# pwrliang/grpc-rdma

Measured on NVIDIA H100. Metric: streaming_payload_GBps_256conns_4MiB, higher is better.
Workload: dtype u8

## Files before the change

grpc-rdma_b200/csrc/b200_block.cuh:

```cuda
#pragma once
#include <cuda_runtime.h>
#include <stdint.h>

#include "b200_dev.cuh"
#include "b200_warp.cuh"

#ifndef VL
#define VL(x) (*(volatile decltype(x)*)&(x))
#endif

#ifndef B200_RECV_PROXY_FENCE
#define B200_RECV_PROXY_FENCE 1
#endif

namespace b200 {


__device__ __forceinline__ uint32_t smem_u32(const void* p) { return (uint32_t)__cvta_generic_to_shared(p); }
__device__ __forceinline__ void mbar_init(uint64_t* bar, uint32_t count) {
  asm volatile("mbarrier.init.shared::cta.b64 [%0], %1;" ::"r"(smem_u32(bar)), "r"(count) : "memory");
}
__device__ __forceinline__ void mbar_expect_tx(uint64_t* bar, uint32_t bytes) {
  asm volatile("mbarrier.arrive.expect_tx.shared::cta.b64 _, [%0], %1;" ::"r"(smem_u32(bar)), "r"(bytes) : "memory");
}
// ... 1 lines not shown
  uint32_t ok;
  asm volatile(
      "{\n\t.reg .pred p;\n\t"
      "mbarrier.try_wait.parity.shared::cta.b64 p, [%1], %2;\n\t"
      "selp.u32 %0, 1, 0, p;\n\t}"
      : "=r"(ok)
      : "r"(smem_u32(bar)), "r"(parity)
      : "memory");
  return ok != 0;
}
__device__ __forceinline__ void bulk_g2s(void* sdst, const void* gsrc, uint32_t bytes, uint64_t* bar) {
  asm volatile("cp.async.bulk.shared::cluster.global.mbarrier::complete_tx::bytes [%0], [%1], %2, [%3];" ::"r"(
                   smem_u32(sdst)),
               "l"(gsrc), "r"(bytes), "r"(smem_u32(bar))
               : "memory");
}
__device__ __forceinline__ void fence_proxy_async_global() { asm volatile("fence.proxy.async.global;" ::: "memory"); }
__device__ __forceinline__ void bulk_s2g(void* gdst, const void* ssrc, uint32_t bytes) {
  asm volatile("cp.async.bulk.global.shared::cta.bulk_group [%0], [%1], %2;" ::"l"(gdst), "r"(smem_u32(ssrc)),
               "r"(bytes)
               : "memory");
}
__device__ __forceinline__ void bulk_commit() { asm volatile("cp.async.bulk.commit_group;" ::: "memory"); }

template <int K>
__device__ __forceinline__ void realign_vectors(uint4* sv, uint32_t nvec, uint32_t r, uint32_t lane) {
  for (uint32_t j = 0; j < nvec; j += 32) {
    const uint32_t i = j + lane;
    uint4 o = make_uint4(0, 0, 0, 0);
    if (i < nvec) {
      const uint4 A = sv[i], B = sv[i + 1];
      uint32_t x0, x1, x2, x3, x4;
      if (K == 0) { x0 = A.x; x1 = A.y; x2 = A.z; x3 = A.w; x4 = B.x; }
      else if (K == 1) { x0 = A.y; x1 = A.z; x2 = A.w; x3 = B.x; x4 = B.y; }
      else if (K == 2) { x0 = A.z; x1 = A.w; x2 = B.x; x3 = B.y; x4 = B.z; }
      else { x0 = A.w; x1 = B.x; x2 = B.y; x3 = B.z; x4 = B.w; }
      o.x = __funnelshift_r(x0, x1, r);
      o.y = __funnelshift_r(x1, x2, r);
      o.z = __funnelshift_r(x2, x3, r);
      o.w = __funnelshift_r(x3, x4, r);
    }
    __syncwarp();
    if (i < nvec) sv[i] = o;
  }
}

__device__ __forceinline__ void smem_to_global(uint8_t* dst, uint8_t* sbase, uint32_t soff, uint32_t n,
                                               uint32_t lane) {
  if (n == 0) return;
  uint32_t head = (16 - (uint32_t)(reinterpret_cast<uintptr_t>(dst) & 15)) & 15;
  if (head > n) head = n;
  const uint32_t nvec = (n - head) >> 4;
  const uint32_t tail = n - head - (nvec << 4);
  if (lane < head) dst[lane] = sbase[soff + lane];
  if (lane < tail) dst[head + (nvec << 4) + lane] = sbase[soff + head + (nvec << 4) + lane];
  if (nvec == 0) return;
  const uint32_t vs = soff + head, m = vs & 15;
  uint4* sv = reinterpret_cast<uint4*>(sbase + (vs - m));
  if (m != 0) {
    __syncwarp();
    const uint32_t r = (m & 3) * 8;
    switch (m >> 2) {
      case 0: realign_vectors<0>(sv, nvec, r, lane); break;
      case 1: realign_vectors<1>(sv, nvec, r, lane); break;
      case 2: realign_vectors<2>(sv, nvec, r, lane); break;
      default: realign_vectors<3>(sv, nvec, r, lane); break;
    }
    asm volatile("fence.proxy.async.shared::cta;" ::: "memory");
    __syncwarp();
  }
  if (lane == 0) bulk_s2g(dst + head, sv, nvec << 4);
}

constexpr uint32_t kZeroBytes = 1024;
__device__ __forceinline__ void coop_zero(uint8_t* p, uint64_t n, const uint8_t* zero, uint32_t lane) {
  if (n == 0) return;
  uint64_t head = (16 - (reinterpret_cast<uintptr_t>(p) & 15)) & 15;
  if (head > n) head = n;
  if (lane < head) p[lane] = 0;
  p += head;
  n -= head;
  const uint64_t body = n & ~15ull;
  if (lane < n - body) p[body + lane] = 0;
  if (lane == 0)
    for (uint64_t o = 0; o < body; o += kZeroBytes)
      bulk_s2g(p + o, zero, body - o < kZeroBytes ? (uint32_t)(body - o) : kZeroBytes);
}


#ifndef B200_MOVERS
#define B200_MOVERS 8
#endif
#ifndef B200_DEPTH
#define B200_DEPTH 3
// ... 110 lines not shown
      bulk_commit();
      *(volatile uint32_t*)&w->ready = 0;
    }
    head++;
  }
  if (lane == 0) {
    asm volatile("cp.async.bulk.wait_group 0;" ::: "memory");
    fence_proxy_async_global();
  }
  __syncwarp();
}


constexpr uint32_t kTiny = 32;
constexpr uint32_t kFootCap = 1024;
__device__ __forceinline__ void foot_put(uint32_t* foot8, bool stamped, uint32_t i, uint64_t off, uint64_t p) {
  if (stamped) reinterpret_cast<uint64_t*>(foot8)[i] = (off >> 3) | p << 32;
  else foot8[i] = (uint32_t)(off >> 3);
}

struct SendPlanState {
  uint64_t rt, cap, staging, total_left, written_total, ncalls, cur, bidx, last_rh;
  uint64_t tx;
  uint32_t partial, max_sge, coalesce, stamped;
};

struct SendCallScratch {
  const uint8_t* src[kMaxSgeLimit];
  uint64_t len[kMaxSgeLimit];
  uint64_t off[kMaxSgeLimit];
  uint32_t first_item[kMaxSgeLimit + 1];
};

template <bool kStamped>
__device__ __noinline__ void send_produce_segment(const SendOpDev& op, const PairDev* P, uint8_t* ring,
                                                  SendPlanState& S, SendCallScratch& CS, WorkItem* q, PipeCtl* ctl,
                                                  uint32_t* foot8, uint32_t* nfoot_out, uint32_t lane) {
  const uint64_t cap = S.cap, mask = cap - 1;
  uint32_t base_item = 0, nfoot = 0;
  bool op_done = false;
  constexpr bool stamped = kStamped;
  const uint32_t fcap = stamped ? kFootCap / 2 : kFootCap;
  while (nfoot + kMaxSgeLimit <= fcap) {
    const uint64_t rt = S.rt, tx0 = S.tx;
    const uint64_t rh = ld_volatile_u64(&P->credit_head);
    if (rh != S.last_rh) {
      if (P->wire != 0) __threadfence_system();
      else __threadfence();
      S.last_rh = rh;
    }
    const uint64_t cur = S.cur, bidx = S.bidx;
    const uint64_t idx = cur + lane;
    const bool valid = lane < S.max_sge && idx < op.nreal;
    const uint8_t* ptr = nullptr;
    uint64_t len = 0;
    if (valid) {
      SliceDev sl = op.slices[idx];
      const uint64_t skip = lane == 0 ? bidx : 0;
      ptr = sl.ptr + skip;
      len = sl.len - skip;
    }
    const uint64_t e = valid ? encoded_size(len) : 0;
// ... 12 lines not shown
    const int nfull = first_bad < 0 ? 32 : first_bad;
    uint64_t p = 0;
    if ((int)lane < nfull) p = len;
    else if ((int)lane == nfull && valid && len != 0) p = room;
    const unsigned fmask = __ballot_sync(0xffffffffu, p != 0);
    const uint32_t nframes = __popc(fmask);
    uint64_t wsum = p, esum = p ? encoded_size(p) : 0;
    const bool tiny = p != 0 && p <= kTiny;
    const uint32_t items = (p && !tiny) ? (uint32_t)((p + kChunk - 1) / kChunk) : 0;
    uint32_t items_incl = items;
    for (int o = 1; o < 32; o <<= 1) {
      uint32_t t = __shfl_up_sync(0xffffffffu, items_incl, o);
      if (lane >= (uint32_t)o) items_incl += t;
    }
    for (int o = 16; o > 0; o >>= 1) {
      wsum += __shfl_xor_sync(0xffffffffu, wsum, o);
      esum += __shfl_xor_sync(0xffffffffu, esum, o);
    }
    const uint32_t nitems = __shfl_sync(0xffffffffu, items_incl, 31);
    const uint64_t cut_p = __shfl_sync(0xffffffffu, p, nfull < 32 ? nfull : 0);
    const uint64_t foff = (rt + a) & mask;
    const uint64_t hdr = frame_header(p, stamped ? stamp_of(tx0 + lane) : 0);
    CS.first_item[lane] = items_incl - items;
    if (p) {
      CS.src[lane] = ptr;
      CS.len[lane] = p;
      CS.off[lane] = foff;
      foot_put(foot8, stamped, nfoot + lane, (foff + 8 + round_up8(p)) & mask, p);
    }
    if (tiny) {
      uint64_t w[kTiny / 8];
#pragma unroll
      for (int k = 0; k < (int)(kTiny / 8); k++) w[k] = 0;
#pragma unroll
      for (int i = 0; i < (int)kTiny; i++)
        if ((uint64_t)i < p) w[i >> 3] |= (uint64_t)__ldg(ptr + i) << (8 * (i & 7));
      *reinterpret_cast<uint64_t*>(ring + foff) = hdr;
#pragma unroll
      for (int k = 0; k < (int)(kTiny / 8); k++)
        if ((uint64_t)(8 * k) < p) *reinterpret_cast<uint64_t*>(ring + ((foff + 8 + 8 * k) & mask)) = w[k];
    }
    if (lane == 0) {
      CS.first_item[32] = nitems;
      S.rt = (rt + esum) & mask;
      S.tx = tx0 + nframes;
      S.partial = wsum < S.total_left;
      S.total_left -= wsum;
      S.written_total += wsum;
      if (wsum) S.ncalls++;
      uint64_t nb = 0;
      if (nfull < 32 && nframes > (uint32_t)nfull) nb = (nfull == 0 ? bidx : 0) + cut_p;
      else if (nfull == 0) nb = bidx;
      S.cur = cur + nfull;
      S.bidx = nb;
    }
    __syncwarp();
    nfoot += nframes;
    const unsigned big = __ballot_sync(0xffffffffu, items > 8);
    if (!big && nitems <= kQI) {
      const uint32_t first = items_incl - items;
      for (uint32_t t = 0; t < items; t++) {
        const uint64_t c0 = (uint64_t)t * kChunk;
        uint64_t n = p - c0;
        if (n > kChunk) n = kChunk;
        publish_item(q, base_item + first + t, reinterpret_cast<uint64_t>(ptr + c0), (foff + 8 + c0) & mask,
                     c0 == 0 ? hdr : 0, (uint32_t)n);
      }
    } else
    for (uint32_t it = lane; it < nitems; it += 32) {
      uint32_t f = 0;
      while (f + 1 < nframes && CS.first_item[f + 1] <= it) f++;
      const uint64_t c0 = (uint64_t)(it - CS.first_item[f]) * kChunk;
      const uint64_t flen = CS.len[f];
      uint64_t n = flen - c0;
      if (n > kChunk) n = kChunk;
      publish_item(q, base_item + it, reinterpret_cast<uint64_t>(CS.src[f] + c0), (CS.off[f] + 8 + c0) & mask,
                   c0 == 0 ? frame_header(flen, stamped ? stamp_of(tx0 + f) : 0) : 0, (uint32_t)n);
    }
    __syncwarp();
    base_item += nitems;
    const bool last = (wsum == 0) || !(op.flags & kFlagUntilBlocked) || S.total_left == 0;
    if (last) {
      op_done = true;
      break;
    }
  }
  if (lane == 0) {
    *nfoot_out = nfoot;
    ctl->total_items = base_item;
    ctl->op_done = op_done ? 1u : 0u;
    __threadfence_block();
    *(volatile uint32_t*)&ctl->seg_done = 1;
  }
  __syncwarp();
}

template <bool kStamped>
__device__ __noinline__ void send_produce_coalesced(const SendOpDev& op, const PairDev* P, uint8_t* ring,
                                                    SendPlanState& S, SendCallScratch& CS, WorkItem* q, PipeCtl* ctl,
                                                    uint32_t* foot8, uint32_t* nfoot_out, uint32_t lane) {
  const uint64_t cap = S.cap, mask = cap - 1;
  uint32_t base_item = 0, nfoot = 0;
  bool op_done = false;
  constexpr bool stamped = kStamped;
  const uint32_t fcap = stamped ? kFootCap / 2 : kFootCap;
  while (nfoot < fcap) {
    const uint64_t rt = S.rt;
    const uint64_t rh = ld_volatile_u64(&P->credit_head);
    if (rh != S.last_rh) {
      if (P->wire != 0) __threadfence_system();
      else __threadfence();
      S.last_rh = rh;
    }
    const uint64_t cur = S.cur, bidx = S.bidx;
    const uint64_t wend = op.nreal < cur + kCoalesceSlices ? op.nreal : cur + kCoalesceSlices;
    const uint64_t ws = calc_writable(S.staging), wf = calc_writable(free_size(cap, rh, rt));
    const uint64_t pmax = ws < wf ? ws : wf;
    uint64_t p = 0;
    for (uint64_t g = cur; g < wend && p < pmax; g += 32) {
      const uint64_t idx = g + lane;
      uint64_t len = idx < wend ? op.slices[idx].len - (idx == cur ? bidx : 0) : 0;
      for (int o = 16; o > 0; o >>= 1) len += __shfl_xor_sync(0xffffffffu, len, o);
      p += len;
    }
    if (p > pmax) p = pmax;
// ... 20 lines not shown
      passed += __popc(__ballot_sync(0xffffffffu, valid && a < p && e <= p));
      const unsigned cm = __ballot_sync(0xffffffffu, valid && a < p && e > p);
      if (cm) {
        nb = __shfl_sync(0xffffffffu, skip + (p - a), __ffs(cm) - 1);
        cut = true;
      }
      const bool tiny = n != 0 && n <= kTiny;
      const uint32_t items = (n && !tiny) ? (uint32_t)((n + kChunk - 1) / kChunk) : 0;
      uint32_t items_incl = items;
      for (int o = 1; o < 32; o <<= 1) {
        const uint32_t t = __shfl_up_sync(0xffffffffu, items_incl, o);
        if (lane >= (uint32_t)o) items_incl += t;
      }
      const uint32_t nitems = __shfl_sync(0xffffffffu, items_incl, 31);
      const uint64_t foff = (rt + 8 + a) & mask;
      if (tiny) {
#pragma unroll 1
        for (uint32_t i = 0; i < (uint32_t)n; i++) ring[(foff + i) & mask] = __ldg(ptr + i);
      }
      CS.first_item[lane] = items_incl - items;
      CS.src[lane] = ptr;
      CS.len[lane] = n;
      CS.off[lane] = foff;
      __syncwarp();
      for (uint32_t it = lane; it < nitems; it += 32) {
        uint32_t f = 0;
        while (f + 1 < 32 && CS.first_item[f + 1] <= it) f++;
        const uint64_t c0 = (uint64_t)(it - CS.first_item[f]) * kChunk;
        uint64_t m = CS.len[f] - c0;
        if (m > kChunk) m = kChunk;
        publish_item(q, base_item + it, reinterpret_cast<uint64_t>(CS.src[f] + c0), (CS.off[f] + c0) & mask, 0,
                     (uint32_t)m);
      }
      __syncwarp();
      base_item += nitems;
      pre = __shfl_sync(0xffffffffu, e, 31);
    }
    if (lane == 0) {
      if (p) {
        *reinterpret_cast<uint64_t*>(ring + rt) = frame_header(p, stamped ? stamp_of(S.tx) : 0);
        foot_put(foot8, stamped, nfoot, (rt + 8 + round_up8(p)) & mask, p);
        S.tx++;
        S.rt = (rt + encoded_size(p)) & mask;
        S.ncalls++;
        S.cur = cur + passed;
        S.bidx = cut ? nb : 0;
      }
      S.partial = p < S.total_left;
      S.total_left -= p;
      S.written_total += p;
    }
    __syncwarp();
    if (p) nfoot++;
    if (p == 0 || !(op.flags & kFlagUntilBlocked) || S.total_left == 0) {
      op_done = true;
      break;
    }
  }
  if (lane == 0) {
    *nfoot_out = nfoot;
    ctl->total_items = base_item;
    ctl->op_done = op_done ? 1u : 0u;
    __threadfence_block();
    *(volatile uint32_t*)&ctl->seg_done = 1;
  }
  __syncwarp();
}

struct SendMove {
  uint8_t* ring;
  uint64_t cap, mask;
  __device__ __forceinline__ void issue(uint64_t a, uint32_t n, uint8_t* stage, uint64_t* bar) const {
    const uint32_t pre = (uint32_t)(a & 15);
    const uint32_t len = (pre + n + 15u) & ~15u;
    mbar_expect_tx(bar, len);
    bulk_g2s(stage, reinterpret_cast<const void*>(a - pre), len, bar);
  }
  __device__ __forceinline__ void process(uint64_t a, uint64_t b, uint64_t c, uint32_t n, uint8_t* stage,
                                          uint32_t lane) const {
    const uint32_t pre = (uint32_t)(a & 15);
    if (c != 0 && lane == 0) *reinterpret_cast<uint64_t*>(ring + ((b + cap - 8) & mask)) = c;
    uint64_t seg1 = cap - b;
    if (seg1 > n) seg1 = n;
    smem_to_global(ring + b, stage, pre, (uint32_t)seg1, lane);
    if (n > seg1) smem_to_global(ring, stage, pre + (uint32_t)seg1, n - (uint32_t)seg1, lane);
  }
};

__device__ __forceinline__ void send_body(PairDev* __restrict__ pairs, const SendOpDev& op, OpResult* result,
                                          PipeSmem& pipe, uint8_t* stage_mem, uint32_t& phase_bits) {
  WorkItem* q = pipe.q;
  PipeCtl& ctl = pipe.ctl;
  uint64_t* bars = pipe.bars;
  __shared__ SendPlanState PS;
  __shared__ SendCallScratch CS;
  __shared__ uint64_t foot_mem[kFootCap / 2];
  uint32_t* foot8 = reinterpret_cast<uint32_t*>(foot_mem);
  __shared__ uint32_t s_nfoot;
  __shared__ unsigned long long s_tx0;
  __shared__ unsigned long long s_total;
  __shared__ uint32_t s_status;
  PairDev* P = &pairs[op.slot];
  const uint32_t tid = threadIdx.x, lane = tid & 31, warp = tid >> 5;

  if (tid < kQI) q[tid].ready = 0;
  if (tid == 0) {
    s_total = 0;
    s_status = *(volatile uint32_t*)&P->status;
    PS.rt = *(volatile uint64_t*)&P->remote_tail;
    PS.cap = *(volatile uint64_t*)&P->cap;
    PS.staging = PS.cap / 2;
    const uint32_t sge = *(volatile uint32_t*)&P->max_sge;
    PS.max_sge = sge & ~kSgeModeBits;
    PS.coalesce = (sge & kSgeCoalesce) != 0;
    PS.stamped = (sge & kSgeStamped) != 0;
    PS.tx = PS.stamped ? VL(pair_seq(pairs, op.slot)->tx) : 0;
    PS.cur = 0;
    PS.bidx = op.byte_idx;
    PS.written_total = 0;
    PS.ncalls = 0;
    PS.partial = *(volatile uint32_t*)&P->partial_write;
    PS.last_rh = ~0ull;
  }
  __syncthreads();
  {
    unsigned long long part = 0;
    for (uint64_t i = tid; i < op.nslices; i += kThreads) part += op.slices[i].len;
    for (int o = 16; o > 0; o >>= 1) part += __shfl_down_sync(0xffffffffu, part, o);
    if (lane == 0 && part) atomicAdd(&s_total, part);
  }
  __syncthreads();
  if (s_status != kStConnected) {
    if (tid == 0) {
      result->bytes = 0;
      result->calls = 0;
    }
    return;
  }
  if (tid == 0) PS.total_left = s_total - op.byte_idx;
  const uint64_t cap = VL(P->cap), mask = cap - 1;
  uint8_t* ring = VL(P->peer_ring);
  const bool sys_scope = VL(P->wire) != 0;

  while (true) {
    if (tid == 0) {
      ctl.next = 0;
      ctl.total_items = 0;
      ctl.seg_done = 0;
      ctl.op_done = 0;
      s_nfoot = 0;
      s_tx0 = PS.tx;
    }
    __syncthreads();
    if (warp == 0) {
      if (PS.stamped) {
        if (PS.coalesce) send_produce_coalesced<true>(op, P, ring, PS, CS, q, &ctl, foot8, &s_nfoot, lane);
        else send_produce_segment<true>(op, P, ring, PS, CS, q, &ctl, foot8, &s_nfoot, lane);
      } else {
        if (PS.coalesce) send_produce_coalesced<false>(op, P, ring, PS, CS, q, &ctl, foot8, &s_nfoot, lane);
        else send_produce_segment<false>(op, P, ring, PS, CS, q, &ctl, foot8, &s_nfoot, lane);
      }
    } else {
      const SendMove mv{ring, cap, mask};
      mover_run(mv, q, &ctl, stage_mem + (warp - 1) * (kDepth * kStageBytes), &bars[(warp - 1) * kDepth], phase_bits, lane);
    }
    if (sys_scope) __threadfence_system();
    else __threadfence();
    __syncthreads();
    const uint32_t nfoot = s_nfoot;
    if (PS.stamped) {
      for (uint32_t i = tid; i < nfoot; i += kThreads) {
        const uint64_t v = foot_mem[i];
        const uint64_t hdr = frame_header(v >> 32, stamp_of(s_tx0 + i));
        *reinterpret_cast<uint64_t*>(ring + ((v & 0xffffffffu) << 3)) = ~hdr;
      }
    } else {
      for (uint32_t i = tid; i < nfoot; i += kThreads)
        *reinterpret_cast<uint64_t*>(ring + ((uint64_t)foot8[i] << 3)) = kFooter;
    }
    const bool done = ctl.op_done != 0;
    __syncthreads();
    if (done) break;
  }
  if (tid == 0) {
    P->remote_tail = PS.rt;
    P->partial_write = PS.partial;
    if (PS.stamped) pair_seq(pairs, op.slot)->tx = PS.tx;
// ... 410 lines not shown
```

grpc-rdma_b200/csrc/b200_dev.cuh:

```cuda
#pragma once
#include <stdint.h>

#if defined(__CUDACC__)
#define B200_HD __host__ __device__ __forceinline__
#else
#define B200_HD inline
#endif

namespace b200 {

constexpr uint64_t kAlign = 8;
constexpr uint64_t kReserved = 24;
constexpr uint64_t kFooter = ~0ull;
constexpr int kMaxSgeLimit = 32;
constexpr uint32_t kCoalesceSlices = 1024;
constexpr uint32_t kSgeCoalesce = 0x80000000u;
constexpr uint32_t kSgeStamped = 0x40000000u;
constexpr uint32_t kSgeModeBits = kSgeCoalesce | kSgeStamped;
constexpr uint64_t kStampMod = (1ull << 24) - 1;
constexpr uint64_t kLenMask = (1ull << 40) - 1;
constexpr uint64_t kStampedMaxCap = 256ull << 20;
constexpr int kMaxPairs = 8192;

B200_HD uint64_t round_up8(uint64_t v) { return (v + 7) & ~7ull; }
B200_HD uint64_t round_down8(uint64_t v) { return v & ~7ull; }
B200_HD uint64_t encoded_size(uint64_t payload) { return 16 + round_up8(payload); }
B200_HD uint64_t calc_writable(uint64_t space) { return space > kReserved ? round_down8(space - kReserved) : 0; }
B200_HD uint64_t free_size(uint64_t cap, uint64_t head, uint64_t tail) {
  return cap - ((tail + cap - head) & (cap - 1));
}
B200_HD uint64_t writable_size(uint64_t cap, uint64_t head, uint64_t tail) {
  uint64_t f = free_size(cap, head, tail);
  return f > kReserved ? f - kReserved : 0;
}

B200_HD uint32_t stamp_of(uint64_t s) { return 1u + (uint32_t)(s % kStampMod); }
B200_HD uint64_t frame_header(uint64_t p, uint32_t st) { return p | (uint64_t)st << 40; }
B200_HD uint64_t frame_footer(uint64_t hdr, uint32_t st) { return st ? ~hdr : kFooter; }
B200_HD uint64_t frame_present(uint64_t hdr, uint64_t cap, uint32_t st) {
  const uint64_t p = st ? hdr & kLenMask : hdr;
  if (st && (uint32_t)(hdr >> 40) != st) return 0;
  return p != 0 && p <= cap - kReserved ? p : 0;
}
B200_HD uint64_t frame_complete(uint64_t hdr, uint64_t foot, uint64_t cap, uint32_t st) {
  const uint64_t p = frame_present(hdr, cap, st);
// ... 140 lines not shown
  uint16_t events;
};
struct SvcPollState {
  uint32_t hi_slot;
  uint32_t stop;
  uint32_t ready_next;
  uint32_t scans;
};
struct SvcParams {
  PairDev* pairs;
  PairSvc* psvc;
  SvcCmd* cmds;
  SvcDone* done;
  BigBox* boxes;
  EagerRec* erec;
  uint8_t* eslots;
  SvcPollState* ps;
  uint32_t* last_ev;
  ReadyEntry* ready;
  uint32_t* host_scans;
  int nowners, nbig;
};

void launch_send(PairDev* pairs, const SendOpDev* ops, OpResult* results, int nops, void* stream);
void launch_recv(PairDev* pairs, const RecvOpDev* ops, OpResult* results, int nops, void* stream);
void launch_poll_scan(PairDev* pairs, const int32_t* slots, uint32_t* events, uint32_t* ready_count,
                      int32_t* ready_slots, int n, void* stream);

bool launch_service(const SvcParams& sp, void* s_owner, void* s_big, void* s_poll);
int svc_trace_read(unsigned long long* out16);

void launch_probe_copy(uint8_t* dst, const uint8_t* src, uint64_t bytes_per_cta, uint64_t stride, int nctas,
                       int threads, uint32_t mis, uint32_t item_bytes, uint32_t dynamic, void* stream);

}
```

grpc-rdma_b200/csrc/b200_kernels.cu:

```cuda
#include <cuda_runtime.h>
#include <stdint.h>

#include <mutex>

#include "b200_dev.cuh"
#include "b200_warp.cuh"
#include "b200_block.cuh"

namespace b200 {


__device__ __forceinline__ uint4 ld_stream16(const void* p) {
  uint4 r;
  asm volatile("ld.global.nc.L1::no_allocate.v4.u32 {%0,%1,%2,%3}, [%4];"
               : "=r"(r.x), "=r"(r.y), "=r"(r.z), "=r"(r.w)
               : "l"(p));
  return r;
}
__device__ __forceinline__ uint4 ld_ring16(const void* p) {
  uint4 r;
  asm volatile("ld.global.L1::no_allocate.v4.u32 {%0,%1,%2,%3}, [%4];"
               : "=r"(r.x), "=r"(r.y), "=r"(r.z), "=r"(r.w)
               : "l"(p));
  return r;
}


__global__ void __launch_bounds__(kThreads, 2)
k_send(PairDev* __restrict__ pairs, const SendOpDev* __restrict__ ops, OpResult* __restrict__ results) {
  extern __shared__ __align__(128) uint8_t stage_mem[];
  __shared__ PipeSmem pipe;
  movers_init(pipe, threadIdx.x);
  uint32_t phase_bits = 0;
  const SendOpDev op = ops[blockIdx.x];
  send_body(pairs, op, &results[blockIdx.x], pipe, stage_mem, phase_bits);
}


__global__ void __launch_bounds__(kThreads, 2)
k_recv(PairDev* __restrict__ pairs, const RecvOpDev* __restrict__ ops, OpResult* __restrict__ results) {
  extern __shared__ __align__(128) uint8_t stage_mem[];
  __shared__ PipeSmem pipe;
  movers_init(pipe, threadIdx.x);
  uint32_t phase_bits = 0;
  const RecvOpDev op = ops[blockIdx.x];
  recv_body(pairs, op, &results[blockIdx.x], pipe, stage_mem, phase_bits);
}


__global__ void __launch_bounds__(128)
k_poll_scan(PairDev* __restrict__ pairs, const int32_t* __restrict__ slots, uint32_t* __restrict__ events,
            uint32_t* __restrict__ ready_count, int32_t* __restrict__ ready_slots, int n) {
  const int i = blockIdx.x * blockDim.x + threadIdx.x;
  const uint32_t lane = threadIdx.x & 31;
  uint32_t ev = 0;
  int32_t slot = -1;
  if (i < n) {
    slot = slots[i];
// ... 885 lines not shown
  ensure_kernel_attrs();
  int dev = 0, sms = 0, per_sm = 0;
  cudaGetDevice(&dev);
  cudaDeviceGetAttribute(&sms, cudaDevAttrMultiProcessorCount, dev);
  if (cudaOccupancyMaxActiveBlocksPerMultiprocessor(&per_sm, k_svc_big, kThreads, kStageTotal) != cudaSuccess ||
      sp.nbig + 2 > per_sm * sms)
    return false;
  const int octas = (sp.nowners + 3) / 4;
  k_svc_owner<<<octas, 128, 0, static_cast<cudaStream_t>(s_owner)>>>(sp);
  k_svc_big<<<sp.nbig, kThreads, kStageTotal, static_cast<cudaStream_t>(s_big)>>>(sp);
  k_svc_poll<<<1, kThreads, 0, static_cast<cudaStream_t>(s_poll)>>>(sp);
  return cudaGetLastError() == cudaSuccess;
}

void launch_probe_copy(uint8_t* dst, const uint8_t* src, uint64_t bytes_per_cta, uint64_t stride, int nctas,
                       int threads, uint32_t mis, uint32_t item_bytes, uint32_t dynamic, void* stream) {
  (void)threads;
  ensure_kernel_attrs();
  k_probe_copy<<<nctas, kThreads, kStageTotal, static_cast<cudaStream_t>(stream)>>>(
      dst, const_cast<uint8_t*>(src), bytes_per_cta, stride, mis, item_bytes, dynamic);
}


void launch_send(PairDev* pairs, const SendOpDev* ops, OpResult* results, int nops, void* stream) {
  if (nops <= 0) return;
  ensure_kernel_attrs();
  k_send<<<nops, kThreads, kStageTotal, static_cast<cudaStream_t>(stream)>>>(pairs, ops, results);
}
void launch_recv(PairDev* pairs, const RecvOpDev* ops, OpResult* results, int nops, void* stream) {
  if (nops <= 0) return;
  ensure_kernel_attrs();
  k_recv<<<nops, kThreads, kStageTotal, static_cast<cudaStream_t>(stream)>>>(pairs, ops, results);
}
void launch_poll_scan(PairDev* pairs, const int32_t* slots, uint32_t* events, uint32_t* ready_count,
                      int32_t* ready_slots, int n, void* stream) {
  if (n <= 0) return;
  ensure_kernel_attrs();
  k_poll_scan<<<(n + 127) / 128, 128, 0, static_cast<cudaStream_t>(stream)>>>(pairs, slots, events, ready_count,
                                                                               ready_slots, n);
}

}
```

grpc-rdma_b200/csrc/b200_runtime.cu:

```cuda
#include <cuda_runtime.h>
#include <errno.h>
#include <poll.h>
#include <stdio.h>
#include <stdlib.h>
#include <string.h>
#include <fcntl.h>
#include <signal.h>
#include <sys/eventfd.h>
#include <sys/stat.h>
#include <unistd.h>

#include <atomic>
#include <chrono>
#include <condition_variable>
#include <map>
#include <mutex>
#include <queue>
#include <string>
#include <thread>
#include <unordered_map>
#include <vector>

#include "../../include/b200_pair.h"
#include "b200_dev.cuh"
// ... 2 lines not shown


static thread_local std::string t_err;
static void set_err(const std::string& s) { t_err = s; }
#define CU_OK(call)                                                                      \
  ([&]() -> bool {                                                                       \
    cudaError_t e__ = (call);                                                            \
    if (e__ != cudaSuccess) {                                                            \
      set_err(std::string(#call) + ": " + cudaGetErrorString(e__));                      \
      return false;                                                                      \
    }                                                                                    \
    return true;                                                                         \
  }())


struct Config {
  uint64_t ring_bytes = 4096ull * 1024;
  int poller_threads = 1;
  int busy_poll_us = 500;
  int poller_sleep_ms = 1000;
  int max_sge = 30;
  int send_coalesce = 0;
  int ring_stamped = 0;
};

struct AddrBlob {
  uint32_t lid;
  uint32_t qpn;
  uint32_t psn;
  uint32_t _pad0;
  uint8_t gid[16];
  uint32_t tag;
  uint32_t _pad1;
  uint64_t ring_buffer_size;
};
static_assert(sizeof(AddrBlob) == B200_ADDRESS_BYTES, "address blob must stay 48 bytes");
constexpr uint32_t kBlobStamped = 0x1;

struct b200_pair {
  int slot = -1;
  int status = B200_UNINITIALIZED;
  std::string id, error;
  uint8_t* ring = nullptr;
  uint64_t cap = 0;
  int wakeup_fd = -1;
  PairMirror* mirror = nullptr;
  AddrBlob self{};
// ... 297 lines not shown
  if (device < 0) {
    const char* e = getenv("B200_DEVICE");
    if (e) device = atoi(e);
    else if (cudaGetDevice(&device) != cudaSuccess) device = 0;
  }
  if (!CU_OK(cudaSetDevice(device))) return -1;
  cudaDeviceProp prop;
  if (!CU_OK(cudaGetDeviceProperties(&prop, device))) return -1;
  if (prop.major != 9 || prop.minor != 0) {
    set_err("b200_init: device is sm_" + std::to_string(prop.major) + std::to_string(prop.minor) +
            ", this library is built for sm_90a only");
    return -1;
  }
  r.dev = device;
  r.cfg.ring_bytes = (uint64_t)env_long("GRPC_RDMA_RING_BUFFER_SIZE_KB", 4096) * 1024;
  if (getenv("B200_RING_BUFFER_SIZE_BYTES")) r.cfg.ring_bytes = (uint64_t)env_long("B200_RING_BUFFER_SIZE_BYTES", 0);
  r.cfg.poller_threads = (int)env_long("GRPC_RDMA_POLLER_THREAD_NUM", 1);
  r.cfg.busy_poll_us = (int)env_long("GRPC_RDMA_BUSY_POLLING_TIMEOUT_US", 500);
  r.cfg.poller_sleep_ms = (int)env_long("GRPC_RDMA_POLLER_SLEEP_TIMEOUT_MS", 1000);
  r.cfg.max_sge = (int)env_long("GRPC_RDMA_MAX_SGE", 30);
  if (r.cfg.max_sge < 1 || r.cfg.max_sge > kMaxSgeLimit) r.cfg.max_sge = 30;
  r.cfg.send_coalesce = env_long("B200_SEND_COALESCE", 0) == 1 ? 1 : 0;
  r.cfg.ring_stamped = env_long("B200_RING_STAMPED", 0) == 1 ? 1 : 0;

  if (!CU_OK(cudaStreamCreateWithFlags(&r.stream, cudaStreamNonBlocking))) return -1;
  if (!CU_OK(cudaStreamCreateWithFlags(&r.poll_stream, cudaStreamNonBlocking))) return -1;
  for (int i = 0; i < kLanes; i++) {
    if (!CU_OK(cudaStreamCreateWithFlags(&r.lane_up[i], cudaStreamNonBlocking))) return -1;
    if (!CU_OK(cudaStreamCreateWithFlags(&r.lane_down[i], cudaStreamNonBlocking))) return -1;
    for (cudaEvent_t* e : {&r.send_done[i], &r.recv_done[i], &r.join_up[i], &r.join_down[i]})
      if (!CU_OK(cudaEventCreateWithFlags(e, cudaEventDisableTiming))) return -1;
  }
  if (!CU_OK(cudaEventCreateWithFlags(&r.fork_event, cudaEventDisableTiming))) return -1;
  const size_t table_bytes = (sizeof(PairDev) + sizeof(PairSeq)) * kMaxPairs;
  if (!CU_OK(cudaMalloc(&r.d_pairs, table_bytes))) return -1;
  if (!CU_OK(cudaMemset(r.d_pairs, 0, table_bytes))) return -1;
  if (!CU_OK(cudaHostAlloc(&r.h_mirrors, sizeof(PairMirror) * kMaxPairs, cudaHostAllocMapped | cudaHostAllocPortable)))
    return -1;
  memset(r.h_mirrors, 0, sizeof(PairMirror) * kMaxPairs);
  auto halloc = [&](void** p, size_t n) {
    return CU_OK(cudaHostAlloc(p, n, cudaHostAllocMapped | cudaHostAllocPortable));
  };
  if (!halloc((void**)&r.h_sop, sizeof(SendOpDev)) || !halloc((void**)&r.h_rop, sizeof(RecvOpDev)) ||
      !halloc((void**)&r.h_slices, sizeof(SliceDev) * (kCoalesceSlices + 1)) ||
      !halloc((void**)&r.h_res, sizeof(OpResult)) ||
      !halloc((void**)&r.h_scan_slots, sizeof(int32_t) * kMaxPairs) ||
// ... 88 lines not shown
    if (v <= 0) return -1;
    r.cfg.ring_bytes = (uint64_t)v * 1024;
  } else if (k == "B200_RING_BUFFER_SIZE_BYTES") {
    if (v <= (long)kReserved) return -1;
    r.cfg.ring_bytes = (uint64_t)v;
  } else if (k == "GRPC_RDMA_POLLER_THREAD_NUM") {
    if (v <= 0) return -1;
    r.cfg.poller_threads = (int)v;
  } else if (k == "GRPC_RDMA_BUSY_POLLING_TIMEOUT_US") {
    if (v < 0) return -1;
    r.cfg.busy_poll_us = (int)v;
  } else if (k == "GRPC_RDMA_POLLER_SLEEP_TIMEOUT_MS") {
    if (v < 0) return -1;
    r.cfg.poller_sleep_ms = (int)v;
  } else if (k == "GRPC_RDMA_MAX_SGE") {
    if (v < 1 || v > kMaxSgeLimit) return -1;
    r.cfg.max_sge = (int)v;
  } else if (k == "B200_SEND_COALESCE") {
    if (v != 0 && v != 1) return -1;
    r.cfg.send_coalesce = (int)v;
  } else if (k == "B200_RING_STAMPED") {
    if (v != 0 && v != 1) return -1;
    r.cfg.ring_stamped = (int)v;
  } else {
    set_err("b200_config_set: unknown key " + k);
    return -1;
  }
  return 0;
}

extern "C" int64_t b200_config_get(const char* key) {
  if (!ensure_init()) return -1;
  Runtime& r = R();
  std::string k(key);
  if (k == "GRPC_RDMA_RING_BUFFER_SIZE_KB") return (int64_t)(r.cfg.ring_bytes / 1024);
  if (k == "B200_RING_BUFFER_SIZE_BYTES") return (int64_t)r.cfg.ring_bytes;
  if (k == "GRPC_RDMA_POLLER_THREAD_NUM") return r.cfg.poller_threads;
  if (k == "GRPC_RDMA_BUSY_POLLING_TIMEOUT_US") return r.cfg.busy_poll_us;
  if (k == "GRPC_RDMA_POLLER_SLEEP_TIMEOUT_MS") return r.cfg.poller_sleep_ms;
  if (k == "GRPC_RDMA_MAX_SGE") return r.cfg.max_sge;
  if (k == "B200_SEND_COALESCE") return r.cfg.send_coalesce;
  if (k == "B200_RING_STAMPED") return r.cfg.ring_stamped;
  return -1;
}


extern "C" void* b200_mem_alloc_device(size_t bytes) {
  if (!ensure_init()) return nullptr;
  void* p = nullptr;
  cudaSetDevice(R().dev);
  if (!CU_OK(cudaMalloc(&p, bytes ? bytes : 1))) return nullptr;
  reg_add(p, bytes ? bytes : 1, 2);
  return p;
}
extern "C" void b200_mem_free_device(void* p) {
  if (!p) return;
  reg_del(p);
  rt_free(p, 0);
}
extern "C" void* b200_mem_alloc_host(size_t bytes) {
  if (!ensure_init()) return nullptr;
  void* p = nullptr;
  cudaSetDevice(R().dev);
  if (!CU_OK(cudaHostAlloc(&p, bytes ? bytes : 1, cudaHostAllocMapped | cudaHostAllocPortable))) return nullptr;
  reg_add(p, bytes ? bytes : 1, 1);
// ... 1009 lines not shown
      memcpy(r.bounce_tx + bounce_off, ptr + skip, take);
      r.h_slices[i].ptr = r.bounce_tx + bounce_off - skip;
      bounce_off += (take + 15) & ~15ull;
    } else {
      r.h_slices[i].ptr = ptr;
    }
    r.h_slices[i].len = len;
  }
  size_t nsl = look;
  if (rest) {
    r.h_slices[nsl].ptr = nullptr;
    r.h_slices[nsl].len = rest;
    nsl++;
  }
  r.h_sop->slot = p->slot;
  const bool conc = p->peer_local && p->peer_local->device_owned.load();
  r.h_sop->flags = B200_BATCH_ONE_CALL | (conc ? B200_BATCH_CONCURRENT : 0);
  r.h_sop->slices = r.h_slices;
  r.h_sop->nslices = nsl;
  r.h_sop->nreal = look;
  r.h_sop->byte_idx = byte_idx;
  r.h_res->bytes = 0;
  r.h_res->calls = 0;
  launch_send(r.d_pairs, r.h_sop, r.h_res, 1, r.stream);
  r.launches++;
  if (!CU_OK(cudaGetLastError()) || !CU_OK(cudaStreamSynchronize(r.stream))) {
    p->error = t_err;
    p->status = B200_ERROR;
    return 0;
  }
  return r.h_res->bytes;
}

extern "C" uint64_t b200_pair_recv(b200_pair* p, void* dst, uint64_t cap) {
  if (!p || !ensure_init()) return 0;
  Runtime& r = R();
  const HostOp op(p);
  if (!op.ok) return 0;
  drain_retire(p);
  if (p->status == B200_CONNECTED && !p->remote && !peer_device_owned(p) &&
      ((volatile PairMirror*)p->mirror)->has_message == 0)
    return 0;
  if (r.svc_running.load()) {
    if (p->status != B200_CONNECTED || cap == 0) return 0;
    return svc_recv(r, p, dst, cap);
  }
  std::lock_guard<std::mutex> lk(r.mu);
// ... 269 lines not shown
  if (!b) return -1;
  Runtime& r = R();
  if (b->nops == 0) return 0;
  if (!b->counted) {
    for (b200_pair* p : b->op_pairs) p->host_ops.fetch_add(1);
    b->counted = true;
  }
  if (any_device_owned((const b200_pair* const*)b->op_pairs.data(), b->op_pairs.size(), sizeof(b200_pair*),
                       "b200_batch_launch")) {
    batch_uncount(b);
    return -1;
  }
  if (!batch_make_concurrent(b)) return -1;
  if (r.svc_running.load()) r.svc_gen++;
  if (b->kind == 1 && r.svc_running.load()) {
    for (b200_pair* p : b->pairs) {
      drain_retire(p);
      ((volatile EagerRec*)&r.svc_erec[p->slot])->magic = 0;
      p->svc_delivered += 1ull << 40;
    }
  }
  if (!b->staged) {
    cudaStream_t s = stream ? (cudaStream_t)stream : r.stream;
    if (b->kind == 0) launch_send(r.d_pairs, (const SendOpDev*)b->d_ops, b->d_results, b->nops, s);
    else launch_recv(r.d_pairs, (const RecvOpDev*)b->d_ops, b->d_results, b->nops, s);
    r.launches++;
    return CU_OK(cudaGetLastError()) ? 0 : -1;
  }
  if (stream && b200_lanes_fork(stream) != 0) return -1;
  for (int L = 0; L < kLanes; L++) {
    LanePlan& lp = b->lanes[L];
    if (lp.nops == 0) continue;
    if (b->kind == 0) {
      cudaStream_t s = r.lane_up[L];
      for (const CopyRun& c : lp.copies)
        if (!CU_OK(cudaMemcpyAsync(c.dst, c.src, c.bytes, cudaMemcpyHostToDevice, s))) return -1;
      if (!CU_OK(cudaStreamWaitEvent(s, r.recv_done[L], 0))) return -1;
      launch_send(r.d_pairs, (const SendOpDev*)b->d_ops + lp.first_op, b->d_results + lp.first_op, lp.nops, s);
      if (!CU_OK(cudaEventRecord(r.send_done[L], s))) return -1;
    } else {
      cudaStream_t s = r.lane_down[L];
      if (!CU_OK(cudaStreamWaitEvent(s, r.send_done[L], 0))) return -1;
      launch_recv(r.d_pairs, (const RecvOpDev*)b->d_ops + lp.first_op, b->d_results + lp.first_op, lp.nops, s);
      if (!CU_OK(cudaEventRecord(r.recv_done[L], s))) return -1;
      for (const CopyRun& c : lp.copies)
        if (!CU_OK(cudaMemcpyAsync(c.dst, c.src, c.bytes, cudaMemcpyDeviceToHost, s))) return -1;
    }
    r.launches++;
    if (!CU_OK(cudaGetLastError())) return -1;
  }
  if (stream && b200_lanes_join(stream) != 0) return -1;
  return 0;
}

extern "C" int b200_batch_results(b200_batch* b, uint64_t* out, void* stream) {
  if (!b) return -1;
  Runtime& r = R();
  if (b->nops == 0) return 0;
  cudaStream_t s = stream ? (cudaStream_t)stream : r.stream;
  if (b->staged) {
    for (int L = 0; L < kLanes; L++)
// ... 589 lines not shown
```

Measured before the change: 524.6.

## Defer publishing first ring window and store it with L2 evict_last hints

```diff
diff --git a/grpc-rdma_b200/csrc/b200_block.cuh b/grpc-rdma_b200/csrc/b200_block.cuh
--- a/grpc-rdma_b200/csrc/b200_block.cuh
+++ b/grpc-rdma_b200/csrc/b200_block.cuh
@@ -47,6 +47,17 @@
                : "memory");
 }
 __device__ __forceinline__ void bulk_commit() { asm volatile("cp.async.bulk.commit_group;" ::: "memory"); }
+
+__device__ __forceinline__ uint64_t l2_policy_evict_last() {
+  uint64_t p;
+  asm volatile("createpolicy.fractional.L2::evict_last.b64 %0, 1.0;" : "=l"(p));
+  return p;
+}
+__device__ __forceinline__ void bulk_s2g_hint(void* gdst, const void* ssrc, uint32_t bytes, uint64_t pol) {
+  asm volatile("cp.async.bulk.global.shared::cta.bulk_group.L2::cache_hint [%0], [%1], %2, %3;" ::"l"(gdst),
+               "r"(smem_u32(ssrc)), "r"(bytes), "l"(pol)
+               : "memory");
+}
 
 template <int K>
 __device__ __forceinline__ void realign_vectors(uint4* sv, uint32_t nvec, uint32_t r, uint32_t lane) {
@@ -70,8 +81,9 @@
   }
 }
 
+template <bool kHint = false>
 __device__ __forceinline__ void smem_to_global(uint8_t* dst, uint8_t* sbase, uint32_t soff, uint32_t n,
-                                               uint32_t lane) {
+                                               uint32_t lane, uint64_t pol = 0) {
   if (n == 0) return;
   uint32_t head = (16 - (uint32_t)(reinterpret_cast<uintptr_t>(dst) & 15)) & 15;
   if (head > n) head = n;
@@ -94,7 +106,10 @@
     asm volatile("fence.proxy.async.shared::cta;" ::: "memory");
     __syncwarp();
   }
-  if (lane == 0) bulk_s2g(dst + head, sv, nvec << 4);
+  if (lane == 0) {
+    if (kHint) bulk_s2g_hint(dst + head, sv, nvec << 4, pol);
+    else bulk_s2g(dst + head, sv, nvec << 4);
+  }
 }
 
 constexpr uint32_t kZeroBytes = 1024;
@@ -251,8 +266,39 @@
 struct SendPlanState {
   uint64_t rt, cap, staging, total_left, written_total, ncalls, cur, bidx, last_rh;
   uint64_t tx;
+  uint64_t win_lo;
+  uint32_t win;
   uint32_t partial, max_sge, coalesce, stamped;
 };
+
+constexpr uint32_t kHoldMax = kL2HandoffMaxKB * 1024 / kChunk;
+struct HeldItem {
+  uint64_t a, b, c;
+  uint32_t n;
+};
+__device__ __forceinline__ uint32_t held_items(uint64_t rel, uint32_t g0, uint32_t items, uint32_t win) {
+  if (items == 0 || rel >= win || g0 >= kHoldMax) return 0;
+  uint32_t h = (uint32_t)((win - rel + kChunk - 1) / kChunk);
+  if (h > items) h = items;
+  if (h > kHoldMax - g0) h = kHoldMax - g0;
+  return h;
+}
+__device__ __forceinline__ uint32_t warp_sum(uint32_t v) {
+  for (int o = 16; o > 0; o >>= 1) v += __shfl_xor_sync(0xffffffffu, v, o);
+  return v;
+}
+__device__ __forceinline__ void emit_item(WorkItem* q, HeldItem* hold, bool held, uint32_t g, uint32_t nheld,
+                                          uint64_t a, uint64_t b, uint64_t c, uint32_t n) {
+  if (held) hold[g] = HeldItem{a, b, c, n};
+  else publish_item(q, g - nheld, a, b, c, n);
+}
+__device__ __forceinline__ void publish_held(WorkItem* q, const HeldItem* hold, uint32_t base_item, uint32_t nheld,
+                                             uint32_t lane) {
+  __syncwarp();
+  for (uint32_t j = lane; j < nheld; j += 32)
+    publish_item(q, base_item - nheld + j, hold[j].a, hold[j].b, hold[j].c, hold[j].n);
+  __syncwarp();
+}
 
 struct SendCallScratch {
   const uint8_t* src[kMaxSgeLimit];
@@ -261,12 +307,15 @@
   uint32_t first_item[kMaxSgeLimit + 1];
 };
 
-template <bool kStamped>
+template <bool kStamped, bool kHold>
 __device__ __noinline__ void send_produce_segment(const SendOpDev& op, const PairDev* P, uint8_t* ring,
                                                   SendPlanState& S, SendCallScratch& CS, WorkItem* q, PipeCtl* ctl,
-                                                  uint32_t* foot8, uint32_t* nfoot_out, uint32_t lane) {
+                                                  uint32_t* foot8, uint32_t* nfoot_out, HeldItem* hold, uint32_t lane) {
   const uint64_t cap = S.cap, mask = cap - 1;
   uint32_t base_item = 0, nfoot = 0;
+  uint32_t nheld = 0;
+  const uint64_t win_lo = S.win_lo;
+  const uint32_t win = S.win;
   bool op_done = false;
   constexpr bool stamped = kStamped;
   const uint32_t fcap = stamped ? kFootCap / 2 : kFootCap;
@@ -325,6 +374,8 @@
     const uint64_t foff = (rt + a) & mask;
     const uint64_t hdr = frame_header(p, stamped ? stamp_of(tx0 + lane) : 0);
     CS.first_item[lane] = items_incl - items;
+    const uint32_t held = held_items((foff + 8 - win_lo) & mask, base_item + items_incl - items, items, win);
+    if (kHold) nheld += warp_sum(held);
     if (p) {
       CS.src[lane] = ptr;
       CS.len[lane] = p;
@@ -366,8 +417,12 @@
         const uint64_t c0 = (uint64_t)t * kChunk;
         uint64_t n = p - c0;
         if (n > kChunk) n = kChunk;
-        publish_item(q, base_item + first + t, reinterpret_cast<uint64_t>(ptr + c0), (foff + 8 + c0) & mask,
-                     c0 == 0 ? hdr : 0, (uint32_t)n);
+        if (kHold)
+          emit_item(q, hold, t < held, base_item + first + t, nheld, reinterpret_cast<uint64_t>(ptr + c0),
+                    (foff + 8 + c0) & mask, c0 == 0 ? hdr : 0, (uint32_t)n);
+        else
+          publish_item(q, base_item + first + t, reinterpret_cast<uint64_t>(ptr + c0), (foff + 8 + c0) & mask,
+                       c0 == 0 ? hdr : 0, (uint32_t)n);
       }
     } else
     for (uint32_t it = lane; it < nitems; it += 32) {
@@ -377,8 +432,13 @@
       const uint64_t flen = CS.len[f];
       uint64_t n = flen - c0;
       if (n > kChunk) n = kChunk;
-      publish_item(q, base_item + it, reinterpret_cast<uint64_t>(CS.src[f] + c0), (CS.off[f] + 8 + c0) & mask,
-                   c0 == 0 ? frame_header(flen, stamped ? stamp_of(tx0 + f) : 0) : 0, (uint32_t)n);
+      if (kHold)
+        emit_item(q, hold, ((CS.off[f] + 8 + c0 - win_lo) & mask) < win && base_item + it < kHoldMax,
+                  base_item + it, nheld, reinterpret_cast<uint64_t>(CS.src[f] + c0), (CS.off[f] + 8 + c0) & mask,
+                  c0 == 0 ? frame_header(flen, stamped ? stamp_of(tx0 + f) : 0) : 0, (uint32_t)n);
+      else
+        publish_item(q, base_item + it, reinterpret_cast<uint64_t>(CS.src[f] + c0), (CS.off[f] + 8 + c0) & mask,
+                     c0 == 0 ? frame_header(flen, stamped ? stamp_of(tx0 + f) : 0) : 0, (uint32_t)n);
     }
     __syncwarp();
     base_item += nitems;
@@ -388,6 +448,10 @@
       break;
     }
   }
+  if (kHold) {
+    publish_held(q, hold, base_item, nheld, lane);
+    if (lane == 0) S.win = 0;
+  }
   if (lane == 0) {
     *nfoot_out = nfoot;
     ctl->total_items = base_item;
@@ -398,12 +462,16 @@
   __syncwarp();
 }
 
-template <bool kStamped>
+template <bool kStamped, bool kHold>
 __device__ __noinline__ void send_produce_coalesced(const SendOpDev& op, const PairDev* P, uint8_t* ring,
                                                     SendPlanState& S, SendCallScratch& CS, WorkItem* q, PipeCtl* ctl,
-                                                    uint32_t* foot8, uint32_t* nfoot_out, uint32_t lane) {
+                                                    uint32_t* foot8, uint32_t* nfoot_out, HeldItem* hold,
+                                                    uint32_t lane) {
   const uint64_t cap = S.cap, mask = cap - 1;
   uint32_t base_item = 0, nfoot = 0;
+  uint32_t nheld = 0;
+  const uint64_t win_lo = S.win_lo;
+  const uint32_t win = S.win;
   bool op_done = false;
   constexpr bool stamped = kStamped;
   const uint32_t fcap = stamped ? kFootCap / 2 : kFootCap;
@@ -470,6 +538,7 @@
       CS.src[lane] = ptr;
       CS.len[lane] = n;
       CS.off[lane] = foff;
+      if (kHold) nheld += warp_sum(held_items((foff - win_lo) & mask, base_item + items_incl - items, items, win));
       __syncwarp();
       for (uint32_t it = lane; it < nitems; it += 32) {
         uint32_t f = 0;
@@ -477,8 +546,12 @@
         const uint64_t c0 = (uint64_t)(it - CS.first_item[f]) * kChunk;
         uint64_t m = CS.len[f] - c0;
         if (m > kChunk) m = kChunk;
-        publish_item(q, base_item + it, reinterpret_cast<uint64_t>(CS.src[f] + c0), (CS.off[f] + c0) & mask, 0,
-                     (uint32_t)m);
+        if (kHold)
+          emit_item(q, hold, ((CS.off[f] + c0 - win_lo) & mask) < win && base_item + it < kHoldMax, base_item + it,
+                    nheld, reinterpret_cast<uint64_t>(CS.src[f] + c0), (CS.off[f] + c0) & mask, 0, (uint32_t)m);
+        else
+          publish_item(q, base_item + it, reinterpret_cast<uint64_t>(CS.src[f] + c0), (CS.off[f] + c0) & mask, 0,
+                       (uint32_t)m);
       }
       __syncwarp();
       base_item += nitems;
@@ -505,6 +578,10 @@
       break;
     }
   }
+  if (kHold) {
+    publish_held(q, hold, base_item, nheld, lane);
+    if (lane == 0) S.win = 0;
+  }
   if (lane == 0) {
     *nfoot_out = nfoot;
     ctl->total_items = base_item;
@@ -524,19 +601,35 @@
     mbar_expect_tx(bar, len);
     bulk_g2s(stage, reinterpret_cast<const void*>(a - pre), len, bar);
   }
-  __device__ __forceinline__ void process(uint64_t a, uint64_t b, uint64_t c, uint32_t n, uint8_t* stage,
-                                          uint32_t lane) const {
+  template <bool kHint = false>
+  __device__ __forceinline__ void store(uint64_t a, uint64_t b, uint64_t c, uint32_t n, uint8_t* stage, uint32_t lane,
+                                        uint64_t pol = 0) const {
     const uint32_t pre = (uint32_t)(a & 15);
     if (c != 0 && lane == 0) *reinterpret_cast<uint64_t*>(ring + ((b + cap - 8) & mask)) = c;
     uint64_t seg1 = cap - b;
     if (seg1 > n) seg1 = n;
-    smem_to_global(ring + b, stage, pre, (uint32_t)seg1, lane);
-    if (n > seg1) smem_to_global(ring, stage, pre + (uint32_t)seg1, n - (uint32_t)seg1, lane);
+    smem_to_global<kHint>(ring + b, stage, pre, (uint32_t)seg1, lane, pol);
+    if (n > seg1) smem_to_global<kHint>(ring, stage, pre + (uint32_t)seg1, n - (uint32_t)seg1, lane, pol);
+  }
+  __device__ __forceinline__ void process(uint64_t a, uint64_t b, uint64_t c, uint32_t n, uint8_t* stage,
+                                          uint32_t lane) const {
+    store(a, b, c, n, stage, lane);
   }
 };
 
+struct SendMoveWin : SendMove {
+  uint64_t win_lo, win_len, pol_last;
+  __device__ __forceinline__ void process(uint64_t a, uint64_t b, uint64_t c, uint32_t n, uint8_t* stage,
+                                          uint32_t lane) const {
+    if (((b - win_lo) & mask) < win_len) store<true>(a, b, c, n, stage, lane, pol_last);
+    else store(a, b, c, n, stage, lane);
+  }
+};
+
+template <bool kHold = false>
 __device__ __forceinline__ void send_body(PairDev* __restrict__ pairs, const SendOpDev& op, OpResult* result,
-                                          PipeSmem& pipe, uint8_t* stage_mem, uint32_t& phase_bits) {
+                                          PipeSmem& pipe, uint8_t* stage_mem, uint32_t& phase_bits,
+                                          HeldItem* hold = nullptr, uint32_t window = 0) {
   WorkItem* q = pipe.q;
   PipeCtl& ctl = pipe.ctl;
   uint64_t* bars = pipe.bars;
@@ -569,6 +662,10 @@
     PS.ncalls = 0;
     PS.partial = *(volatile uint32_t*)&P->partial_write;
     PS.last_rh = ~0ull;
+    if (kHold) {
+      PS.win_lo = PS.rt;
+      PS.win = window;
+    }
   }
   __syncthreads();
   {
@@ -601,16 +698,31 @@
     }
     __syncthreads();
     if (warp == 0) {
-      if (PS.stamped) {
-        if (PS.coalesce) send_produce_coalesced<true>(op, P, ring, PS, CS, q, &ctl, foot8, &s_nfoot, lane);
-        else send_produce_segment<true>(op, P, ring, PS, CS, q, &ctl, foot8, &s_nfoot, lane);
+      if (kHold && PS.win != 0) {
+        if (PS.stamped) {
+          if (PS.coalesce) send_produce_coalesced<true, true>(op, P, ring, PS, CS, q, &ctl, foot8, &s_nfoot, hold, lane);
+          else send_produce_segment<true, true>(op, P, ring, PS, CS, q, &ctl, foot8, &s_nfoot, hold, lane);
+        } else {
+          if (PS.coalesce) send_produce_coalesced<false, true>(op, P, ring, PS, CS, q, &ctl, foot8, &s_nfoot, hold, lane);
+          else send_produce_segment<false, true>(op, P, ring, PS, CS, q, &ctl, foot8, &s_nfoot, hold, lane);
+        }
+      } else if (PS.stamped) {
+        if (PS.coalesce) send_produce_coalesced<true, false>(op, P, ring, PS, CS, q, &ctl, foot8, &s_nfoot, nullptr, lane);
+        else send_produce_segment<true, false>(op, P, ring, PS, CS, q, &ctl, foot8, &s_nfoot, nullptr, lane);
       } else {
-        if (PS.coalesce) send_produce_coalesced<false>(op, P, ring, PS, CS, q, &ctl, foot8, &s_nfoot, lane);
-        else send_produce_segment<false>(op, P, ring, PS, CS, q, &ctl, foot8, &s_nfoot, lane);
+        if (PS.coalesce) send_produce_coalesced<false, false>(op, P, ring, PS, CS, q, &ctl, foot8, &s_nfoot, nullptr, lane);
+        else send_produce_segment<false, false>(op, P, ring, PS, CS, q, &ctl, foot8, &s_nfoot, nullptr, lane);
       }
     } else {
-      const SendMove mv{ring, cap, mask};
-      mover_run(mv, q, &ctl, stage_mem + (warp - 1) * (kDepth * kStageBytes), &bars[(warp - 1) * kDepth], phase_bits, lane);
+      if (kHold) {
+        const SendMoveWin mv{{ring, cap, mask}, PS.win_lo, window, l2_policy_evict_last()};
+        mover_run(mv, q, &ctl, stage_mem + (warp - 1) * (kDepth * kStageBytes), &bars[(warp - 1) * kDepth], phase_bits,
+                  lane);
+      } else {
+        const SendMove mv{ring, cap, mask};
+        mover_run(mv, q, &ctl, stage_mem + (warp - 1) * (kDepth * kStageBytes), &bars[(warp - 1) * kDepth], phase_bits,
+                  lane);
+      }
     }
     if (sys_scope) __threadfence_system();
     else __threadfence();
diff --git a/grpc-rdma_b200/csrc/b200_dev.cuh b/grpc-rdma_b200/csrc/b200_dev.cuh
--- a/grpc-rdma_b200/csrc/b200_dev.cuh
+++ b/grpc-rdma_b200/csrc/b200_dev.cuh
@@ -21,6 +21,8 @@
 constexpr uint64_t kLenMask = (1ull << 40) - 1;
 constexpr uint64_t kStampedMaxCap = 256ull << 20;
 constexpr int kMaxPairs = 8192;
+constexpr int kL2HandoffMaxKB = 256;
+constexpr int kL2HandoffDefaultKB = 128;
 
 B200_HD uint64_t round_up8(uint64_t v) { return (v + 7) & ~7ull; }
 B200_HD uint64_t round_down8(uint64_t v) { return v & ~7ull; }
@@ -207,7 +209,7 @@
   int nowners, nbig;
 };
 
-void launch_send(PairDev* pairs, const SendOpDev* ops, OpResult* results, int nops, void* stream);
+void launch_send(PairDev* pairs, const SendOpDev* ops, OpResult* results, int nops, void* stream, uint32_t window);
 void launch_recv(PairDev* pairs, const RecvOpDev* ops, OpResult* results, int nops, void* stream);
 void launch_poll_scan(PairDev* pairs, const int32_t* slots, uint32_t* events, uint32_t* ready_count,
                       int32_t* ready_slots, int n, void* stream);
diff --git a/grpc-rdma_b200/csrc/b200_kernels.cu b/grpc-rdma_b200/csrc/b200_kernels.cu
--- a/grpc-rdma_b200/csrc/b200_kernels.cu
+++ b/grpc-rdma_b200/csrc/b200_kernels.cu
@@ -26,14 +26,16 @@
 }
 
 
-__global__ void __launch_bounds__(kThreads, 2)
-k_send(PairDev* __restrict__ pairs, const SendOpDev* __restrict__ ops, OpResult* __restrict__ results) {
+__global__ void __maxnreg__(80)
+k_send(PairDev* __restrict__ pairs, const SendOpDev* __restrict__ ops, OpResult* __restrict__ results,
+       uint32_t window) {
   extern __shared__ __align__(128) uint8_t stage_mem[];
   __shared__ PipeSmem pipe;
+  __shared__ HeldItem hold[kHoldMax];
   movers_init(pipe, threadIdx.x);
   uint32_t phase_bits = 0;
   const SendOpDev op = ops[blockIdx.x];
-  send_body(pairs, op, &results[blockIdx.x], pipe, stage_mem, phase_bits);
+  send_body<true>(pairs, op, &results[blockIdx.x], pipe, stage_mem, phase_bits, hold, window);
 }
 
 
@@ -965,10 +967,10 @@
 }
 
 
-void launch_send(PairDev* pairs, const SendOpDev* ops, OpResult* results, int nops, void* stream) {
+void launch_send(PairDev* pairs, const SendOpDev* ops, OpResult* results, int nops, void* stream, uint32_t window) {
   if (nops <= 0) return;
   ensure_kernel_attrs();
-  k_send<<<nops, kThreads, kStageTotal, static_cast<cudaStream_t>(stream)>>>(pairs, ops, results);
+  k_send<<<nops, kThreads, kStageTotal, static_cast<cudaStream_t>(stream)>>>(pairs, ops, results, window);
 }
 void launch_recv(PairDev* pairs, const RecvOpDev* ops, OpResult* results, int nops, void* stream) {
   if (nops <= 0) return;
diff --git a/grpc-rdma_b200/csrc/b200_runtime.cu b/grpc-rdma_b200/csrc/b200_runtime.cu
--- a/grpc-rdma_b200/csrc/b200_runtime.cu
+++ b/grpc-rdma_b200/csrc/b200_runtime.cu
@@ -48,7 +48,9 @@
   int max_sge = 30;
   int send_coalesce = 0;
   int ring_stamped = 0;
+  int l2_handoff_kb = kL2HandoffDefaultKB;
 };
+bool l2_handoff_ok(long kb) { return kb >= 0 && kb <= kL2HandoffMaxKB; }
 
 struct AddrBlob {
   uint32_t lid;
@@ -392,6 +394,10 @@
   if (r.cfg.max_sge < 1 || r.cfg.max_sge > kMaxSgeLimit) r.cfg.max_sge = 30;
   r.cfg.send_coalesce = env_long("B200_SEND_COALESCE", 0) == 1 ? 1 : 0;
   r.cfg.ring_stamped = env_long("B200_RING_STAMPED", 0) == 1 ? 1 : 0;
+  {
+    const long kb = env_long("B200_L2_HANDOFF_KB", kL2HandoffDefaultKB);
+    r.cfg.l2_handoff_kb = l2_handoff_ok(kb) ? (int)kb : kL2HandoffDefaultKB;
+  }
 
   if (!CU_OK(cudaStreamCreateWithFlags(&r.stream, cudaStreamNonBlocking))) return -1;
   if (!CU_OK(cudaStreamCreateWithFlags(&r.poll_stream, cudaStreamNonBlocking))) return -1;
@@ -526,6 +532,9 @@
   } else if (k == "B200_RING_STAMPED") {
     if (v != 0 && v != 1) return -1;
     r.cfg.ring_stamped = (int)v;
+  } else if (k == "B200_L2_HANDOFF_KB") {
+    if (!l2_handoff_ok(v)) return -1;
+    r.cfg.l2_handoff_kb = (int)v;
   } else {
     set_err("b200_config_set: unknown key " + k);
     return -1;
@@ -545,6 +554,7 @@
   if (k == "GRPC_RDMA_MAX_SGE") return r.cfg.max_sge;
   if (k == "B200_SEND_COALESCE") return r.cfg.send_coalesce;
   if (k == "B200_RING_STAMPED") return r.cfg.ring_stamped;
+  if (k == "B200_L2_HANDOFF_KB") return r.cfg.l2_handoff_kb;
   return -1;
 }
 
@@ -1600,7 +1610,7 @@
   r.h_sop->byte_idx = byte_idx;
   r.h_res->bytes = 0;
   r.h_res->calls = 0;
-  launch_send(r.d_pairs, r.h_sop, r.h_res, 1, r.stream);
+  launch_send(r.d_pairs, r.h_sop, r.h_res, 1, r.stream, 0);
   r.launches++;
   if (!CU_OK(cudaGetLastError()) || !CU_OK(cudaStreamSynchronize(r.stream))) {
     p->error = t_err;
@@ -1916,7 +1926,7 @@
   }
   if (!b->staged) {
     cudaStream_t s = stream ? (cudaStream_t)stream : r.stream;
-    if (b->kind == 0) launch_send(r.d_pairs, (const SendOpDev*)b->d_ops, b->d_results, b->nops, s);
+    if (b->kind == 0) launch_send(r.d_pairs, (const SendOpDev*)b->d_ops, b->d_results, b->nops, s, r.cfg.l2_handoff_kb * 1024u);
     else launch_recv(r.d_pairs, (const RecvOpDev*)b->d_ops, b->d_results, b->nops, s);
     r.launches++;
     return CU_OK(cudaGetLastError()) ? 0 : -1;
@@ -1930,7 +1940,8 @@
       for (const CopyRun& c : lp.copies)
         if (!CU_OK(cudaMemcpyAsync(c.dst, c.src, c.bytes, cudaMemcpyHostToDevice, s))) return -1;
       if (!CU_OK(cudaStreamWaitEvent(s, r.recv_done[L], 0))) return -1;
-      launch_send(r.d_pairs, (const SendOpDev*)b->d_ops + lp.first_op, b->d_results + lp.first_op, lp.nops, s);
+      launch_send(r.d_pairs, (const SendOpDev*)b->d_ops + lp.first_op, b->d_results + lp.first_op, lp.nops, s,
+                  r.cfg.l2_handoff_kb * 1024u);
       if (!CU_OK(cudaEventRecord(r.send_done[L], s))) return -1;
     } else {
       cudaStream_t s = r.lane_down[L];
```

Measured after the change: 526.4, median of 6. No clear change (+0.3%).
